# charlie-foxtrot/RTLSDR-Airband

Measured on AMD Instinct MI355X. Metric: IQ Msamples/sec channelized+demodulated per node; % HBM roofline, higher is better.
Workload: dtype i8x3->i32->f32 (stage 1), f32 (stage 2)

## Files before the change

### rtlsdr-airband_amd/_build.py

```python
from __future__ import annotations

import os
import subprocess
import sys

import hashlib

HERE = os.path.dirname(os.path.abspath(__file__))
CSRC = os.path.join(HERE, "csrc")
ARCH = "gfx950"
EXTRA = os.environ.get("AIRBAND_EXTRA_DEFINES", "").split()
TAG = os.environ.get("AIRBAND_BUILD_TAG") or (hashlib.sha1(" ".join(EXTRA).encode()).hexdigest()[:8] if EXTRA else "")
OBJ = os.path.join(HERE, "build" + ("_exp_" + TAG if EXTRA else ""))
LIB = os.path.join(HERE, "libairband_hip" + ("_exp_" + TAG if EXTRA else "") + ".so")

DEVICE_FLAGS = ["-Xclang", "-target-feature", "-Xclang", "-packed-fp32-ops"]

HIP_SOURCES = {
    "channelizer_fft.hip": ["-O3"],
    "channelizer_dft.hip": ["-O3"],
    "channelizer_dft_wide.hip": ["-O3"],
    "channelizer_f32.hip": ["-O3"],
    "misc_kernels.hip": ["-O3", "-ffp-contract=off"],
    "demod.hip": ["-O3", "-ffp-contract=off", "-fhip-fp32-correctly-rounded-divide-sqrt"],
    "gate.hip": ["-O3"],
    "airband_hip.cpp": ["-O2", "-x", "hip"],
}
HOST_SOURCES = {"params.cpp": ["-O2", "-ffp-contract=off", "-fno-fast-math"]}


def _newer(src: str, dst: str) -> bool:
    if not os.path.exists(dst):
        return True
    t = os.path.getmtime(dst)
    deps = [src, os.path.abspath(__file__)] + [os.path.join(CSRC, f) for f in os.listdir(CSRC) if f.endswith(".h")] + [os.path.join(HERE, "..", "include", "airband_hip.h")]
    return any(os.path.getmtime(d) > t for d in deps)


def _run(cmd):
    r = subprocess.run(cmd, stdout=subprocess.PIPE, stderr=subprocess.STDOUT, text=True)
    if r.returncode != 0:
        sys.stderr.write(" ".join(cmd) + "\n" + r.stdout)
        raise RuntimeError("build failed: " + " ".join(cmd[:3]))
    return r.stdout


LLVM_BIN = "/opt/rocm/lib/llvm/bin"
FORBIDDEN = r"^\s+v_pk_(mul|fma|add)_f32"


def device_disassembly(lib: str):
    import re
    import shutil
    import tempfile

    def tool(name):
        t = os.path.join(LLVM_BIN, name)
        t = t if os.path.exists(t) else shutil.which(name)
        if not t:
            raise RuntimeError("the packed-f32 guard needs " + name + " (ROCm's llvm/bin)")
        return t

    units = []
    with tempfile.TemporaryDirectory(prefix="airband_fatbin_") as d:
        fat = os.path.join(d, "fat.bin")
        _run([tool("llvm-objcopy"), "--dump-section", ".hip_fatbin=" + fat, lib, os.devnull])
        blob = open(fat, "rb").read()
        magic = b"__CLANG_OFFLOAD_BUNDLE__"
        starts = [m.start() for m in re.finditer(re.escape(magic), blob)]
        if not starts:
            raise RuntimeError("no offload bundle in .hip_fatbin of " + lib)
        for n, (a, b) in enumerate(zip(starts, starts[1:] + [len(blob)])):
            piece, co = os.path.join(d, "bundle%d.bin" % n), os.path.join(d, "unit%d.co" % n)
            open(piece, "wb").write(blob[a:b])
            _run([tool("clang-offload-bundler"), "--unbundle", "--type=o", "--targets=hipv4-amdgcn-amd-amdhsa--" + ARCH, "--input=" + piece, "--output=" + co])
            text = _run([tool("llvm-objdump"), "-d", co])
            units.append((re.findall(r"^[0-9a-f]+ <(\w+)>:", text, re.M), text))
    return units


def check_no_packed_f32(lib: str) -> int:
    import re

    n = 0
    for kernels, text in device_disassembly(lib):
        for line in text.split("\n"):
            if re.match(r"^\s+[sv]_\w+|^\s+(ds|global|buffer|flat|scratch)_\w+", line):
                n += 1
                if re.match(FORBIDDEN, line):
                    raise RuntimeError("packed-f32 instruction in the device code of %s (kernels of the unit: %s ...): %s" % (lib, ", ".join(kernels[:3]), line.strip()))
    if n < 100000 and not EXTRA:
        raise RuntimeError("packed-f32 guard: only %d device instructions found in %s" % (n, lib))
    return n


def build(force: bool = False, verbose: bool = False) -> str:
    sources = [os.path.join(CSRC, name) for name in list(HIP_SOURCES) + list(HOST_SOURCES)]
    if not force and all(os.path.exists(s) for s in sources) and not any(_newer(s, LIB) for s in sources):
        return LIB
    os.makedirs(OBJ, exist_ok=True)
    hipcc = os.environ.get("HIPCC", "/opt/rocm/bin/hipcc")
    objs = []
    changed = False
    for name, flags in HIP_SOURCES.items():
        src = os.path.join(CSRC, name)
        if not os.path.exists(src):
            continue
        obj = os.path.join(OBJ, name + ".o")
        objs.append(obj)
        if force or _newer(src, obj):
            info = ["-DAB_BUILD_DEFINES=\"%s\"" % " ".join(EXTRA)] if name == "airband_hip.cpp" else []
            cmd = [hipcc, "--offload-arch=" + ARCH, "-std=c++17", "-fPIC", "-Wall", "-Wno-unused-function"] + flags + DEVICE_FLAGS + EXTRA + info + ["-c", src, "-o", obj]
            if verbose:
                print(" ".join(cmd))
            _run(cmd)
            changed = True
    for name, flags in HOST_SOURCES.items():
        src = os.path.join(CSRC, name)
        obj = os.path.join(OBJ, name + ".o")
        objs.append(obj)
        if force or _newer(src, obj):
            cmd = ["g++", "-std=c++17", "-fPIC", "-Wall"] + flags + ["-c", src, "-o", obj]
            if verbose:
                print(" ".join(cmd))
            _run(cmd)
            changed = True
    if changed or not os.path.exists(LIB):
        cmd = [hipcc, "--offload-arch=" + ARCH, "-shared", "-fPIC", "-o", LIB] + objs + ["-Wl,--no-undefined"]
        if verbose:
            print(" ".join(cmd))
        tmp = LIB + ".unchecked"
        cmd[cmd.index("-o") + 1] = tmp
        _run(cmd)
        if not any("+packed-fp32-ops" in e for e in EXTRA):
            try:
                check_no_packed_f32(tmp)
            except Exception:
                os.unlink(tmp)
                raise
        os.replace(tmp, LIB)
    return LIB


if __name__ == "__main__":
    print(build(force="--force" in sys.argv, verbose=True))
```

### rtlsdr-airband_amd/csrc/demod.hip

```cpp
#include <hip/hip_runtime.h>

#include <cstdlib>
#include <type_traits>

#include "common.h"
#include "kernels.h"
#include "squelch_fsm.h"
#include "exact_math.h"

namespace airband {

namespace {

#if !defined(AB_NEEDED_NOW)
#if defined(__HIPCC__)
#define AB_NEEDED_NOW(...) asm volatile("" ::__VA_ARGS__)
#define AB_V(x) "v"(x)
#else
#define AB_NEEDED_NOW(...) ((void)0)
#define AB_V(x) 0
#endif
#endif
#if !defined(AB_SCHED_FENCE)
#if defined(__has_builtin) && __has_builtin(__builtin_amdgcn_sched_barrier)
// ... 57 lines not shown
    int stride;
    int j0;
    const float* stage_base;
    const int* ext_of;
    float* out_wave;
    int wave_stride;
    bool coop;
    int* skip_of;
};

struct RowZero {
    int held;
    bool run_open;
    bool batch_open;
};
__device__ __forceinline__ bool row_skip_run(const RowZero& z) { return (z.held & 2) && !z.run_open; }
__device__ __forceinline__ void row_run_done(RowZero& z) {
    z.batch_open = z.batch_open || z.run_open;
    z.run_open = false;
}

__device__ __forceinline__ void wave_tail_copy(float* row, int B) {
    typedef float v4f __attribute__((ext_vector_type(4)));
    const v4f* src = reinterpret_cast<const v4f*>(row + B);
    v4f* dst = reinterpret_cast<v4f*>(row);
    static_assert((AB_AGC_EXTRA / 4) % 5 == 0, "whole rounds");
#pragma unroll 1
    for (int c = 0; c < AB_AGC_EXTRA / 4; c += 5) {
        const v4f t0 = src[c], t1 = src[c + 1], t2 = src[c + 2], t3 = src[c + 3], t4 = src[c + 4];
        dst[c] = t0; dst[c + 1] = t1; dst[c + 2] = t2; dst[c + 3] = t3; dst[c + 4] = t4;
    }
}

__device__ __forceinline__ void row_tail_copy(RowZero& z, float* row, int B) {
    if ((z.held & 3) != 3) wave_tail_copy(row, B);
    z.held = (z.held & 2) ? 3 : 0;
}

__device__ __forceinline__ void wave_flush(const WaveRow& w, RowZero& z, int n = RUN) {
    const bool skip = row_skip_run(z);
    row_run_done(z);
    if (w.coop) {
        const int lane = threadIdx.x & 63, q = lane & 7;
        AB_LOCKSTEP();
        w.skip_of[lane] = skip ? 1 : 0;
        AB_LOCKSTEP();
        if (4 * q < n) {
#pragma unroll
            for (int i = 0; i < 8; i++) {
                const int c = i * 8 + (lane >> 3);
                if (w.skip_of[c]) continue;
                const float* src = w.stage_base + (4 * q) * OSTRIDE + c;
                float4* dst = reinterpret_cast<float4*>(w.out_wave + (long)w.ext_of[c] * w.wave_stride + AB_OUT_PAD + AB_AGC_EXTRA + w.j0 + 4 * q);
                *dst = make_float4(src[0], src[OSTRIDE], src[2 * OSTRIDE], src[3 * OSTRIDE]);
            }
        }
        AB_LOCKSTEP();
        return;
    }
    if (skip) return;
    float4* dst = reinterpret_cast<float4*>(w.row + AB_AGC_EXTRA + w.j0);
#pragma unroll
    for (int q = 0; q < RUN / 4; q++)
        if (4 * q < n)
        dst[q] = make_float4(w.staged[(4 * q) * w.stride], w.staged[(4 * q + 1) * w.stride], w.staged[(4 * q + 2) * w.stride], w.staged[(4 * q + 3) * w.stride]);
}

__device__ __forceinline__ void emit_sample(const DemodArgs& a, const ChanConst& cc, OutRegs& o, const WaveRow& w, RowZero& z, float2* iqout, uint8_t* trace, int j, bool audio, bool fade,
                                            bool tone, int state, float out, float re, float im, bool write_iq_always) {
    constexpr long S = AB_SLOT_BLOCK;
    if (AB_UNLIKELY(fade)) {
        z.run_open = true;
        float prev = w.row[j];
#pragma nounroll
        for (int k = j + 1; k < j + AB_AGC_EXTRA; k++) {
            prev = prev * 0.94f;
            const int i = k - AB_AGC_EXTRA - w.j0;
            if (i >= 0)
                w.staged[i * w.stride] = prev;
            else
                w.row[k] = prev;
        }
    }
    const bool open = audio && tone;
    if (open) {
        if (cc.flags & AB_F_NOTCH) {
            o.nx0 = o.nx1; o.nx1 = o.nx2; o.nx2 = out;
            o.ny0 = o.ny1; o.ny1 = o.ny2;
            o.ny2 = cc.notch_d0 * o.nx2 - cc.notch_d1 * o.nx1 + cc.notch_d0 * o.nx0 + cc.notch_d1 * o.ny1 - cc.notch_d2 * o.ny0;
            out = o.ny2;
        }
        out *= cc.ampfactor;
        out = (out != out) ? 0.0f : __builtin_amdgcn_fmed3f(out, -1.0f, 1.0f);
        o.axc = '*';
        z.run_open = true;
    } else {
        out = 0.0f;
    }
    w.staged[(j - w.j0) * w.stride] = out;
    if (cc.flags & AB_F_IQ_OUT) {
        if (open) {
            if (write_iq_always) iqout[(long)j * S] = make_float2(re, im);
        } else {
            iqout[(long)j * S] = make_float2(0.0f, 0.0f);
        }
    }
    if (trace) trace[(long)j * S] = (uint8_t)((state & 7) | (open ? 8 : 0) | (audio ? 16 : 0) | (((cc.flags & AB_F_CTCSS) && tone) ? 32 : 0));
}

constexpr unsigned KIND_MASK = AB_F_NFM | AB_F_RAW_IQ | AB_F_LOWPASS | AB_F_CTCSS | AB_F_IQ_OUT;
template <int KIND>
struct KindBits {
    static constexpr unsigned value = KIND == AB_KIND_NFM           ? (AB_F_NFM | AB_F_RAW_IQ)
                                      : KIND == AB_KIND_NFM_LOWPASS ? (AB_F_NFM | AB_F_RAW_IQ | AB_F_LOWPASS)
                                      : KIND == AB_KIND_NFM_CTCSS   ? (AB_F_NFM | AB_F_RAW_IQ | AB_F_CTCSS)
                                                                    : 0u;
};

template <int KIND, bool WAVE_HAS_CTCSS, int W>
__device__ __forceinline__ void demod_wave(const DemodArgs& a, ChanConst cc, ChanState* sp, int slot, const float2* lut, float* ostage, const int* ext_of, int* skip_of, const int* slot_of,
                                           bool full_block) {
    const int lane = threadIdx.x & 63;
    constexpr long S = AB_SLOT_BLOCK;
    const int R = a.ring_rows, B = a.wave_batch;
    const bool valid = (cc.flags & AB_F_VALID) != 0;
    if (KIND != AB_KIND_GENERIC) cc.flags = (cc.flags & ~KIND_MASK) | KindBits<KIND>::value;

    if (!valid) return;

    const bool nfm = cc.flags & AB_F_NFM, raw_iq = cc.flags & AB_F_RAW_IQ, lowpass = cc.flags & AB_F_LOWPASS;
    const lmask m_am = ab_ballot(!nfm), m_raw_iq = ab_ballot(raw_iq);

    Lane L;
    L.m_lowpass = ab_ballot(lowpass);
    L.m_manual = ab_ballot((cc.flags & AB_F_MANUAL) != 0);
    L.manual_level = cc.sq_manual_level;
    L.normal_ratio = cc.sq_normal_ratio;
    L.flappy_ratio = cc.sq_flappy_ratio;
    L.m_flappy_lower = ab_ballot(cc.sq_flappy_ratio < cc.sq_normal_ratio);
    L.sqbuf = a.sqbuf + ab_ring_base(slot, AB_SQ_BUF);
    L.S = S;
    L.prefetched_delay = (KIND == AB_KIND_NFM_LOWPASS);
    L.track_delay_line = (KIND == AB_KIND_NFM_LOWPASS || KIND == AB_KIND_GENERIC);
    L.may_post_filter = (KIND == AB_KIND_NFM_LOWPASS || KIND == AB_KIND_GENERIC);
    L.all_lowpass = (KIND == AB_KIND_NFM_LOWPASS);
    L.shadow_delay = (KIND == AB_KIND_NFM_LOWPASS);

    SqRegs s;
    sq_load(s, L, sp, true);
    const bool aligned4 = ((s.sample_count + 1u) & 3u) == 0u;
    SqShadow sh = {sp->sh_nf, sp->sh_cap, sp->sh_capped};
    const bool first_batch = a.tail_copy == 0;
    s.dly = KIND == AB_KIND_NFM_LOWPASS ? sp->sh_dly : 0.0f;
    float agc = sp->agcavgfast, pr = sp->pr, pj = sp->pj, prev_out = sp->prev_waveout;
    unsigned dm_phi = sp->dm_phi;
    OutRegs o;
    o.nx0 = sp->nx[0]; o.nx1 = sp->nx[1]; o.nx2 = sp->nx[2]; o.ny0 = sp->ny[0]; o.ny1 = sp->ny[1]; o.ny2 = sp->ny[2];
    o.axc = ' ';
    float lxr1 = sp->lxr[1], lxr2 = sp->lxr[2], lxi1 = sp->lxi[1], lxi2 = sp->lxi[2];
    float lyr1 = sp->lyr[1], lyr2 = sp->lyr[2], lyi1 = sp->lyi[1], lyi2 = sp->lyi[2];

    const float one_minus_alpha = 1.0f - cc.alpha;
    const float div_lo = cc.lp_rgain != 0.0f ? AB_DIV_CONST_LO : __builtin_inff();

    float* mag = a.mag + ab_tile_base(slot, R / AB_TILE_ROWS);
    const float2* iqin = a.iq + ab_tile_base(slot, R / AB_TILE_ROWS);
    const int ext = a.slot_to_ext[slot];
    WaveRow wrow;
    wrow.row = a.out_wave + (long)ext * a.wave_stride + AB_OUT_PAD;
    wrow.stride = OSTRIDE;
    wrow.j0 = 0;
    wrow.stage_base = ostage;
    wrow.ext_of = ext_of;
    wrow.out_wave = a.out_wave;
    wrow.wave_stride = a.wave_stride;
    wrow.coop = full_block;
    wrow.skip_of = skip_of;
    lmask audio_seen = 0;
    RowZero rz = {sp->row_zero, false, false};
    float2* iqout = a.iq_out + ab_ring_base(slot, B);
    uint8_t* trace = a.trace ? a.trace + ab_ring_base(slot, B) : nullptr;
    wrow.staged = ostage + lane;
    if (!WAVE_HAS_CTCSS && a.tail_copy) row_tail_copy(rz, wrow.row, B);
    constexpr bool PACKED = WAVE_HAS_CTCSS && KIND == AB_KIND_NFM_CTCSS;
    float2* ct_af = (WAVE_HAS_CTCSS && !PACKED) ? a.ct_af + (long)(slot - a.ct_gen_first_block * 64) * B : nullptr;
    unsigned* ct_ap = PACKED ? a.ct_ap + (long)(slot - a.ct_pk_first_block * 64) * a.ct_pk_pitch : nullptr;
    constexpr int HAND_RUN = PACKED ? RUN : 16;
    float2* hand_base = reinterpret_cast<float2*>(ostage);
    float2* hand = hand_base + lane;
    unsigned* handw_base = reinterpret_cast<unsigned*>(ostage);
    unsigned* handw = handw_base + lane;
    auto ct_row = [&](int c) { return a.ct_af + (long)(slot_of[c] - a.ct_gen_first_block * 64) * B; };
    auto ct_roww = [&](int c) { return a.ct_ap + (long)(slot_of[c] - a.ct_pk_first_block * 64) * a.ct_pk_pitch; };
    auto hand_flush = [&](int n, int jstart) {
        if (PACKED) {
            if (full_block) {
                const int q = lane & 7;
                AB_LOCKSTEP();
                if (4 * q < n) {
#pragma unroll
                    for (int i0 = 0; i0 < 8; i0++) {
#if defined(AB_FLUSH_REVERSED)
                        const int i = 7 - i0;
#else
                        const int i = i0;
#endif
                        const int c = i * 8 + (lane >> 3);
                        const unsigned* src = handw_base + (4 * q) * OSTRIDE + c;
                        *reinterpret_cast<uint4*>(ct_roww(c) + jstart + 4 * q) = make_uint4(src[0], src[OSTRIDE], src[2 * OSTRIDE], src[3 * OSTRIDE]);
                    }
                }
                AB_LOCKSTEP();
            } else {
                for (int i = 0; i < n; i += 4)
                    *reinterpret_cast<uint4*>(ct_ap + jstart + i) = make_uint4(handw[i * OSTRIDE], handw[(i + 1) * OSTRIDE], handw[(i + 2) * OSTRIDE], handw[(i + 3) * OSTRIDE]);
            }
            return;
        }
        if (full_block) {
            const int q = lane & 7;
            AB_LOCKSTEP();
            if (2 * q < n) {
#pragma unroll
                for (int i = 0; i < 8; i++) {
                    const int c = i * 8 + (lane >> 3);
                    const float2 p0 = hand_base[(2 * q) * OSTRIDE + c], p1 = hand_base[(2 * q + 1) * OSTRIDE + c];
                    *reinterpret_cast<float4*>(ct_row(c) + jstart + 2 * q) = make_float4(p0.x, p0.y, p1.x, p1.y);
                }
            }
            AB_LOCKSTEP();
        } else {
            for (int i = 0; i < n; i += 2) {
                const float2 p0 = hand[i * OSTRIDE], p1 = hand[(i + 1) * OSTRIDE];
                *reinterpret_cast<float4*>(ct_af + jstart + i) = make_float4(p0.x, p0.y, p1.x, p1.y);
            }
        }
    };

    constexpr int GS = 4;
    constexpr int GQ = GS / 4;
#if defined(AB_MASKED_DELAY)
    constexpr bool MASKD = KIND == AB_KIND_AM || KIND == AB_KIND_NFM || KIND == AB_KIND_NFM_CTCSS;
#define AB_MD_PARAM , const int r
#define AB_MD_ARG(r) , r
#else
#define AB_MD_PARAM
#define AB_MD_ARG(r)
#endif
    struct Group {
        float4 mc[GQ], md[GQ], c01[GQ], c23[GQ], q01[GQ], q23[GQ];
#if defined(AB_MASKED_DELAY)
        lmask real;
#endif
    };
    auto fetch = [&](Group& q, int j0, int tail0) {
#if defined(AB_MASKED_DELAY)
        const lmask need = MASKD ? (~s.cC & s.active) : ~(lmask)0;
        const bool real_lane = !MASKD || ab_lane(need);
        q.real = need;
#endif
#pragma unroll
        for (int g = 0; g < GQ; g++) {
            const int rc = ring_row(a.row0 + AB_AGC_EXTRA + j0 + 4 * g, R);
#if defined(AB_MASKED_DELAY)
            const int rd = real_lane ? ring_row(a.row0 + j0 + 4 * g, R) : rc;
#else
            const int rd = ring_row(a.row0 + j0 + 4 * g, R);
#endif
            if (!nfm) {
                q.mc[g] = *reinterpret_cast<const float4*>(mag + ab_tile_off(rc));
                q.md[g] = *reinterpret_cast<const float4*>(mag + ab_tile_off(rd));
            } else {
                const float4* cp = reinterpret_cast<const float4*>(iqin + ab_tile_off(rc));
                q.c01[g] = cp[0];
                q.c23[g] = cp[1];
            }
            if (raw_iq) {
                const float4* qp = reinterpret_cast<const float4*>(iqin + ab_tile_off(rd));
                q.q01[g] = qp[0];
                q.q23[g] = qp[1];
            }
        }
        (void)tail0;
    };
#if defined(AB_MASKED_DELAY)
    float g_md[4] = {0.0f, 0.0f, 0.0f, 0.0f}, g_qr[4] = {0.0f, 0.0f, 0.0f, 0.0f}, g_qi[4] = {0.0f, 0.0f, 0.0f, 0.0f};
    lmask g_real = 0;
    int g_jq = 0;
    auto refetch = [&](const lmask miss) {
        if (ab_lane(miss)) {
            const int rd = ring_row(a.row0 + g_jq, R);
            if (!nfm) {
                const float4 v = *reinterpret_cast<const float4*>(mag + ab_tile_off(rd));
                g_md[0] = v.x; g_md[1] = v.y; g_md[2] = v.z; g_md[3] = v.w;
            } else {
                const float4* qp = reinterpret_cast<const float4*>(iqin + ab_tile_off(rd));
                const float4 u = qp[0], v = qp[1];
                g_qr[0] = u.x; g_qi[0] = u.y; g_qr[1] = u.z; g_qi[1] = u.w;
                g_qr[2] = v.x; g_qi[2] = v.y; g_qr[3] = v.z; g_qi[3] = v.w;
            }
        }
        g_real |= miss;
    };
#endif
    auto touch = [&](const Group& q) {
#pragma unroll
        for (int g = 0; g < GQ; g++) {
            if (!nfm) AB_NEEDED_NOW(AB_V(q.mc[g].x), AB_V(q.mc[g].y), AB_V(q.mc[g].z), AB_V(q.mc[g].w), AB_V(q.md[g].x), AB_V(q.md[g].y), AB_V(q.md[g].z), AB_V(q.md[g].w));
            else AB_NEEDED_NOW(AB_V(q.c01[g].x), AB_V(q.c01[g].y), AB_V(q.c01[g].z), AB_V(q.c01[g].w), AB_V(q.c23[g].x), AB_V(q.c23[g].y), AB_V(q.c23[g].z), AB_V(q.c23[g].w));
            if (raw_iq) AB_NEEDED_NOW(AB_V(q.q01[g].x), AB_V(q.q01[g].y), AB_V(q.q01[g].z), AB_V(q.q01[g].w), AB_V(q.q23[g].x), AB_V(q.q23[g].y), AB_V(q.q23[g].z), AB_V(q.q23[g].w));
        }
    };
    auto tail_in = [&](int n) {
// ... 263 lines not shown
                const float xr0 = xr1, xi0 = xi1;
                xr1 = xr2; xi1 = xi2;
                ab_div_const2(tr, ti, cc.lp_gain, cc.lp_rgain, div_lo, xr2, xi2);
                const float yr0 = yr1, yi0 = yi1;
                yr1 = yr2; yi1 = yi2;
                yr2 = (xr0 + xr2) + (2.0f * xr1) + (cc.lp_yc0 * yr0) + (cc.lp_yc1 * yr1);
                yi2 = (xi0 + xi2) + (2.0f * xi1) + (cc.lp_yc0 * yi0) + (cc.lp_yc1 * yi1);
                re = yr2;
                im = yi2;
                fmag = ab_sqrt_rn(re * re + im * im);
            }
            fre[r] = re;
            fim[r] = im;
            if (ab_any(filt)) {
                const float delayed = t.dly;
                const lmask run = filt & ~(t.cOg & ab_ballot(t.delay < AB_SQ_BUF));
                const lmask seed = run & t.cOg & ab_ballot(t.delay == AB_SQ_BUF);
                float full = ab_lane(seed) ? delayed : t.post_full, capped = ab_lane(seed) ? delayed : t.post_capped;
                t.using_post |= run;
                sq_avg(t.cap, full, capped, fmag);
                t.post_full = ab_lane(run) ? full : t.post_full;
                t.post_capped = ab_lane(run) ? capped : t.post_capped;
                bad |= run & ab_ballot(capped < delayed);
            }
            AB_SCHED_FENCE();
        }
        bad |= t.cC & ~ab_ballot(t.closed_count < 1000u) & t.recent_nz;
        if (AB_UNLIKELY(ab_any(bad & t.active))) return false;
        s = t;
        dm_phi = phi;
        lxr1 = xr1; lxr2 = xr2; lxi1 = xi1; lxi2 = xi2; lyr1 = yr1; lyr2 = yr2; lyi1 = yi1; lyi2 = yi2;
        const bool audio = ab_lane(sq_should_audio(s));
        const int state = !a.trace ? 0 : sq_cur(s);
#pragma unroll
        for (int r = 0; r < 4; r++) {
            float out = 0.0f;
            const float re = fre[r], im = fim[r];
            if (audio) {
                if (!(cc.flags & AB_F_QUADRI)) {
                    const float nbj = -pj;
                    const float cr = re * pr - im * nbj;
                    const float cj = im * pr + re * nbj;
                    out = (float)((double)fast_atan2_dev(cj, cr) * 0.31830988618379067154);
                } else {
                    out = (float)((double)((pr * im - re * pj) / (re * re + im * im + 1.0f)) * 0.31830988618379067154);
                }
                pr = re;
                pj = im;
                agc = agc * 0.995f + out * 0.005f;
                out -= agc;
                out = out * one_minus_alpha + prev_out * cc.alpha;
                prev_out = out;
            }
            emit_sample(a, cc, o, wrow, rz, iqout, trace, jq + r, audio, false, true, state, out, re, im, true);
            AB_SCHED_FENCE();
        }
        return true;
    };
    auto group = [&](const Group& q, int j0) {
#pragma unroll
        for (int g = 0; g < GQ; g++) {
            float mcs[4], mds[4] = {0.0f, 0.0f, 0.0f, 0.0f}, qr[4] = {0.0f, 0.0f, 0.0f, 0.0f}, qi[4] = {0.0f, 0.0f, 0.0f, 0.0f};
            if (!nfm) {
                mcs[0] = q.mc[g].x; mcs[1] = q.mc[g].y; mcs[2] = q.mc[g].z; mcs[3] = q.mc[g].w;
                mds[0] = q.md[g].x; mds[1] = q.md[g].y; mds[2] = q.md[g].z; mds[3] = q.md[g].w;
            } else {
                const float pw[4] = {q.c01[g].x * q.c01[g].x + q.c01[g].y * q.c01[g].y, q.c01[g].z * q.c01[g].z + q.c01[g].w * q.c01[g].w,
                                     q.c23[g].x * q.c23[g].x + q.c23[g].y * q.c23[g].y, q.c23[g].z * q.c23[g].z + q.c23[g].w * q.c23[g].w};
                ab_sqrt_rn4(pw, mcs);
            }
            if (raw_iq) {
                qr[0] = q.q01[g].x; qi[0] = q.q01[g].y; qr[1] = q.q01[g].z; qi[1] = q.q01[g].w;
                qr[2] = q.q23[g].x; qi[2] = q.q23[g].y; qr[3] = q.q23[g].z; qi[3] = q.q23[g].w;
            }
            const int jq = j0 + 4 * g;
            if (KIND == AB_KIND_NFM_LOWPASS) {
                const unsigned c0 = s.sample_count;
                const float dpw[4] = {qr[0] * qr[0] + qi[0] * qi[0], qr[1] * qr[1] + qi[1] * qi[1], qr[2] * qr[2] + qi[2] * qi[2], qr[3] * qr[3] + qi[3] * qi[3]};
                float dmag[4];
                ab_sqrt_rn4(dpw, dmag);
#pragma unroll
                for (int r = 0; r < 4; r++) {
                    const int j = jq + r;
                    mds[r] = (first_batch && j < 101) ? 0.0f : sq_shadow_value(sh);
                    if (!(first_batch && j < AB_AGC_EXTRA)) sq_shadow_step(sh, L, dmag[r], c0 + (unsigned)r + 2u);
                }
            }
            if ((jq % RUN) == 0) wrow.j0 = jq;
#if defined(AB_MASKED_DELAY)
            if (MASKD) {
#pragma unroll
                for (int r = 0; r < 4; r++) { g_md[r] = mds[r]; g_qr[r] = qr[r]; g_qi[r] = qi[r]; }
                g_real = q.real;
                g_jq = jq;
                const lmask want0 = nfm ? ((~s.cC | ~s.nC) & ~s.cA & s.active) : (s.cO | s.cCg | s.nO | s.nCg);
                const lmask miss0 = want0 & ~g_real;
                if (AB_UNLIKELY(ab_any(miss0))) refetch(miss0);
                if (SPEC4 && AB_LIKELY(aligned4 && sq_stable4(s))) {
                    if (AB_LIKELY(sq_raw_stable4(s, L, mcs))) {
                        stable_tail4(jq, mcs, g_md, g_qr, g_qi);
                        continue;
                    }
                }
#pragma unroll
                for (int r = 0; r < 4; r++) sample(jq + r, mcs[r], g_md[r], g_qr[r], g_qi[r], r == 0, r);
                continue;
            }
#endif
            if (SPEC4 && AB_LIKELY(aligned4 && sq_stable4(s))) {
                if (AB_LIKELY(sq_raw_stable4(s, L, mcs))) {
                    stable_tail4(jq, mcs, mds, qr, qi);
                    continue;
                }
            }
            if (SPEC4_LP && AB_LIKELY(aligned4 && sq_stable4(s))) {
                if (AB_LIKELY(lp_stable4(jq, mcs, mds, qr, qi))) continue;
            }
#pragma unroll
            for (int r = 0; r < 4; r++) sample(jq + r, mcs[r], mds[r], qr[r], qi[r], r == 0 AB_MD_ARG(r));
        }
    };
    auto flush = [&](int j0) {
        if (!WAVE_HAS_CTCSS && ((j0 + GS) % RUN) == 0) wave_flush(wrow, rz);
        if (WAVE_HAS_CTCSS && ((j0 + GS) % HAND_RUN) == 0) hand_flush(HAND_RUN, j0 + GS - HAND_RUN);
    };

    Group qa, qb;
    fetch(qa, 0, s.tail);
    touch(qa);
    for (int j0 = 0; j0 < B; j0 += 2 * GS) {
#if !defined(AB_REGROUP_FREE)
        if (W > 1 && a.regroup != 2) __syncthreads();
#endif
        fetch(qb, j0 + GS, tail_in(GS));
        group(qa, j0);
        touch(qb);
        flush(j0);
        fetch(qa, j0 + 2 * GS < B ? j0 + 2 * GS : B - GS, tail_in(GS));
        group(qb, j0 + GS);
        touch(qa);
        flush(j0 + GS);
    }

    if (!WAVE_HAS_CTCSS && (B % RUN) != 0) wave_flush(wrow, rz, B % RUN);
    if (WAVE_HAS_CTCSS && (B % HAND_RUN) != 0) hand_flush(B % HAND_RUN, B - B % HAND_RUN);
    if (!WAVE_HAS_CTCSS) {
        if (o.axc != ' ') sp->active_counter++;
        sp->axc_prev = sp->axc;
        sp->axc = o.axc;
        a.out_axc[ext] = (uint8_t)o.axc;
        sp->nx[0] = o.nx0; sp->nx[1] = o.nx1; sp->nx[2] = o.nx2; sp->ny[0] = o.ny0; sp->ny[1] = o.ny1; sp->ny[2] = o.ny2;
        sp->row_zero = rz.batch_open ? 0 : ((rz.held & 1) | 2);
    }
    sp->agcavgfast = agc; sp->pr = pr; sp->pj = pj; sp->prev_waveout = prev_out; sp->dm_phi = dm_phi;
    if (KIND == AB_KIND_NFM_LOWPASS) { sp->sh_nf = sh.nf; sp->sh_cap = sh.cap; sp->sh_capped = sh.capped; sp->sh_dly = s.dly; }
    if (KIND == AB_KIND_GENERIC) sp->sh_dly = sq_delayed(s, L);
    sq_store(s, L, sp, B);
    if (WAVE_HAS_CTCSS) a.sq_key[slot] = ab_lane(audio_seen) ? 1 : 0;
    sp->lxr[1] = lxr1; sp->lxr[2] = lxr2; sp->lxi[1] = lxi1; sp->lxi[2] = lxi2;
    sp->lyr[1] = lyr1; sp->lyr[2] = lyr2; sp->lyi[1] = lyi1; sp->lyi[2] = lyi2;
}

constexpr int TONE_GROUP = 50;

}

#ifndef AB_AM_WAVES_N
#define AB_AM_WAVES_N 4
#endif
constexpr int AB_DEMOD_WAVES = 3, AB_AM_WAVES = AB_AM_WAVES_N, AB_FRONT_WAVES = 3;

constexpr int AB_REGROUP_WAVES = 4;
constexpr int WAVE_LDS_FLOATS = RUN * OSTRIDE + 3 * 64;

template <int W>
__device__ __forceinline__ int wg_regroup(int key, int wave, int lane, int home, int nb, int* slot_at, int* wcnt) {
    const lmask m0 = __ballot(key == 0), m1 = __ballot(key == 1), m2 = __ballot(key == 2);
    if (lane == 0) {
        wcnt[2 * wave] = __builtin_popcountll(m0);
        wcnt[2 * wave + 1] = __builtin_popcountll(m1);
    }
    __syncthreads();
    int tot0 = 0, tot1 = 0, off0 = 0, off1 = 0;
#pragma unroll
    for (int w = 0; w < W; w++) {
        const int c0 = wcnt[2 * w], c1 = wcnt[2 * w + 1];
        tot0 += c0;
        tot1 += c1;
        off0 += w < wave ? c0 : 0;
        off1 += w < wave ? c1 : 0;
    }
    const lmask below = lane == 0 ? 0ull : (~0ull >> (64 - lane));
    const int at = key == 0   ? off0 + __builtin_popcountll(m0 & below)
                   : key == 1 ? tot0 + off1 + __builtin_popcountll(m1 & below)
                   : key == 2 ? tot0 + tot1 + (wave * 64 - off0 - off1) + __builtin_popcountll(m2 & below)
                              : -1;
    if (at >= 0) slot_at[at] = home;
    __syncthreads();
    const int p = wave * 64 + lane;
    return p < nb * 64 ? slot_at[p] : -1;
}

template <int KIND, bool WAVE_HAS_CTCSS, int W>
__device__ __forceinline__ void demod_block(const DemodArgs& a, int first_block, int n_blocks, float* lds_demod) {
    const int lane = threadIdx.x & 63;
    const int wave = W > 1 ? __builtin_amdgcn_readfirstlane((int)(threadIdx.x >> 6)) : 0;
    float2* lut = reinterpret_cast<float2*>(lds_demod);
    if (KIND != AB_KIND_AM) {
        for (int i = threadIdx.x; i < 257; i += 64 * W) lut[i] = make_float2(a.sin_lut[i], a.cos_lut[i]);
        if (W == 1) __syncthreads();
    }
    float* areas = reinterpret_cast<float*>(lut + (KIND == AB_KIND_AM ? 0 : 258));
    float* ostage = areas + wave * WAVE_LDS_FLOATS;
    int* ext_of = reinterpret_cast<int*>(ostage + RUN * OSTRIDE);
    int* skip_of = ext_of + 64;
    int* slot_of = skip_of + 64;
    int slot;
    if (W == 1) {
        slot = (first_block + blockIdx.x) * 64 + lane;
        if (a.perm) slot = a.perm[slot];
    } else {
        int* slot_at = reinterpret_cast<int*>(areas + W * WAVE_LDS_FLOATS);
        int* wcnt = slot_at + W * 64;
        const int block0 = first_block + blockIdx.x * W;
        const int left = first_block + n_blocks - block0, nb = left < W ? left : W;
        const int home = (block0 + wave) * 64 + lane;
        int key = 3;
        if (wave < nb) {
            const ChanState* hp = a.cs + home;
            const bool valid = (a.cc[home].flags & AB_F_VALID) != 0;
            bool busy = valid && (hp->cur != AB_ST_CLOSED || hp->next != AB_ST_CLOSED);
            if (a.regroup == 2) {
                constexpr int G = (KIND == AB_KIND_AM || KIND == AB_KIND_GENERIC) ? 4 : 2;
                const lmask any_busy = __ballot(busy);
                const lmask gmask = ((1ull << G) - 1ull) << (lane & ~(G - 1));
                busy = (any_busy & gmask) != 0ull;
            }
            key = !valid ? 2 : busy ? 0 : 1;
        }
        slot = wg_regroup<W>(key, wave, lane, home, nb, slot_at, wcnt);
        if (slot < 0) return;
    }
    const ChanConst cc = a.cc[slot];
    ext_of[lane] = a.slot_to_ext[slot];
    slot_of[lane] = slot;
    const bool full_block = __ballot((cc.flags & AB_F_VALID) != 0) == ~0ull;
    if (W == 1) __syncthreads();
    else AB_LOCKSTEP_FENCED();
    demod_wave<KIND, WAVE_HAS_CTCSS, W>(a, cc, a.cs + slot, slot, lut, ostage, ext_of, skip_of, slot_of, full_block);
}

template <int KIND, bool WAVE_HAS_CTCSS, int W>
__global__ __launch_bounds__(64 * W, KIND == AB_KIND_AM ? AB_AM_WAVES : KIND == AB_KIND_NFM_CTCSS ? AB_FRONT_WAVES : AB_DEMOD_WAVES) void demod_kernel(DemodArgs a, int first_block, int n_blocks) {
    AB_DYNAMIC_LDS(float, lds_demod);
    demod_block<KIND, WAVE_HAS_CTCSS, W>(a, first_block, n_blocks, lds_demod);
}

constexpr int AB_PERM_WAVES = 16;
template <int G>
__global__ __launch_bounds__(64 * AB_PERM_WAVES) void regroup_perm_kernel(DemodArgs a, int first_block, int n_blocks) {
    __shared__ int slot_at[AB_PERM_WAVES * 64];
    __shared__ int wcnt[AB_PERM_WAVES * 2];
    const int lane = threadIdx.x & 63;
    const int wave = __builtin_amdgcn_readfirstlane((int)(threadIdx.x >> 6));
    const int block0 = first_block + blockIdx.x * AB_PERM_WAVES;
    const int left = first_block + n_blocks - block0, nb = left < AB_PERM_WAVES ? left : AB_PERM_WAVES;
    const int home = (block0 + wave) * 64 + lane;
    int key = 3;
    if (wave < nb) {
        const ChanState* hp = a.cs + home;
        const bool valid = (a.cc[home].flags & AB_F_VALID) != 0;
        const bool busy1 = valid && (hp->cur != AB_ST_CLOSED || hp->next != AB_ST_CLOSED);
        const lmask any_busy = __ballot(busy1);
        const lmask gmask = ((1ull << G) - 1ull) << (lane & ~(G - 1));
        key = !valid ? 2 : (any_busy & gmask) != 0ull ? 0 : 1;
    }
    const int slot = wg_regroup<AB_PERM_WAVES>(key, wave, lane, home, nb, slot_at, wcnt);
    if (slot >= 0) a.perm[home] = slot;
}

#if defined(AB_TONE_WAVES8)
#define AB_TONE_RESIDENCY __attribute__((amdgpu_waves_per_eu(8, 8)))
#else
#define AB_TONE_RESIDENCY
#endif
template <bool PACKED>
__global__ __launch_bounds__(256) AB_TONE_RESIDENCY void tone_kernel(DemodArgs a, int first_block, int n_blocks) {
    __shared__ float power[4][64];
    __shared__ __attribute__((aligned(16))) float xs_all[4][64];
    const int wave = __builtin_amdgcn_readfirstlane((int)((blockIdx.x * blockDim.x + threadIdx.x) >> 6));
    const int lane = threadIdx.x & 63;
    if (wave >= n_blocks * 64) return;
    const int slot = first_block * 64 + wave;
    const unsigned flags = a.cc[slot].flags;
    if (!(flags & AB_F_VALID) || !(flags & AB_F_CTCSS)) return;
    const ChanConst cc = a.cc[slot];
    ChanState* sp = a.cs + slot;
    float* scratch = power[threadIdx.x >> 6];
    float* xs = xs_all[threadIdx.x >> 6];
    const int B = a.wave_batch, NG = B / TONE_GROUP;
    int enough0 = sp->ct_enough[0], enough1 = sp->ct_enough[1], count0 = sp->ct_count[0], count1 = sp->ct_count[1];
    int has0 = sp->ct_has_tone[0], has1 = sp->ct_has_tone[1];
    unsigned found0 = sp->ct_found[0], found1 = sp->ct_found[1], nf0 = sp->ct_not_found[0], nf1 = sp->ct_not_found[1];
    const int n0 = cc.ct_ntones[0], n1 = cc.ct_ntones[1], win0 = cc.ct_window[0], win1 = cc.ct_window[1];
    const float* ctab = a.ct_coeff + (long)cc.ct_slot * 2 * AB_MAX_TONES;
    float* qtab = a.ct_q + (long)cc.ct_slot * 4 * AB_MAX_TONES;
    const bool merged = n0 + n1 <= 64;
    const int fi = merged ? lane - n1 : lane;
    const bool t0 = fi >= 0 && fi < n0, t1 = lane < n1;
    const int fbase = merged ? n1 : 0;
    const float c0 = t0 ? ctab[fi] : 0.0f, c1 = t1 ? ctab[AB_MAX_TONES + lane] : 0.0f;
    float q1f = t0 ? qtab[fi] : 0.0f, q2f = t0 ? qtab[AB_MAX_TONES + fi] : 0.0f;
    float q1s = t1 ? qtab[2 * AB_MAX_TONES + lane] : 0.0f, q2s = t1 ? qtab[3 * AB_MAX_TONES + lane] : 0.0f;

    const long blk = (wave >> 6) + (first_block - a.ct_first_block);
    if (!a.sq_key[slot]) {
        const unsigned long long standing = ((sp->ct_enough[1] ? sp->ct_has_tone[1] : sp->ct_has_tone[0]) != 0) ? ~0ull : 0ull;
        unsigned long long* mp = a.ct_mask + (blk * (a.wave_batch / TONE_GROUP)) * AB_SLOT_BLOCK + (wave & 63);
        if (lane < a.wave_batch / TONE_GROUP) mp[(long)lane * AB_SLOT_BLOCK] = standing;
        return;
    }
    const long hrow = wave + (long)(first_block - (PACKED ? a.ct_pk_first_block : a.ct_gen_first_block)) * 64;
    const float2* af = PACKED ? nullptr : a.ct_af + hrow * B;
    const unsigned* ap = PACKED ? a.ct_ap + hrow * a.ct_pk_pitch : nullptr;
    unsigned long long* maskp = a.ct_mask + (blk * NG) * AB_SLOT_BLOCK + (wave & 63);
    constexpr int DEPTH = 10;
    const int ldlane = lane < TONE_GROUP ? lane : TONE_GROUP - 1;
    auto fetch = [&](int g) {
        const int i = (g < NG ? g : NG - 1) * TONE_GROUP + ldlane;
        if (PACKED) return make_float2(__uint_as_float(ap[i]), 0.0f);
        return af[i];
    };
    float2 ahead[DEPTH];
#pragma unroll
    for (int k = 0; k < DEPTH; k++) ahead[k] = fetch(k);
    unsigned long long verdict[DEPTH];
    auto step = [&](const int g, const float2 got, unsigned long long& mask_out) {
        float2 cur = lane < TONE_GROUP ? got : make_float2(0.0f, 0.0f);
        if (PACKED) {
            const unsigned w = lane < TONE_GROUP ? __float_as_uint(got.x) : HAND_IDLE;
            const bool au = hand_is_audio(w);
            cur = make_float2(au ? __uint_as_float(w) : 0.0f, __uint_as_float(au ? FL_AUDIO : ((w & 1u) ? FL_RESET : 0u)));
        }
        const float ax = cur.x;
        const unsigned fl = __float_as_uint(cur.y);
        unsigned long long mask = 0;
        const bool idle = __ballot((fl & (FL_AUDIO | FL_RESET)) != 0) == 0ull;
        const bool all_audio = __ballot(lane < TONE_GROUP && (fl & (FL_AUDIO | FL_RESET)) != FL_AUDIO) == 0ull;
        if (idle) {
            mask = (enough1 ? has1 : has0) ? ~0ull : 0ull;
        } else if (all_audio && count1 + TONE_GROUP < win1 && (enough1 || count0 + TONE_GROUP < win0)) {
#if defined(AB_TONE_READLANE)
            if (enough1) {
                for (int u = 0; u < TONE_GROUP; u++) {
                    const float x = __uint_as_float(__builtin_amdgcn_readlane(__float_as_uint(ax), u));
                    const float q0 = c1 * q1s - q2s + x;
                    q2s = q1s;
                    q1s = q0;
                }
            } else {
                for (int u = 0; u < TONE_GROUP; u++) {
                    const float x = __uint_as_float(__builtin_amdgcn_readlane(__float_as_uint(ax), u));
                    const float q0 = c1 * q1s - q2s + x;
                    q2s = q1s;
                    q1s = q0;
                    const float p0 = c0 * q1f - q2f + x;
                    q2f = q1f;
                    q1f = p0;
                }
                count0 += TONE_GROUP;
            }
#else
            AB_LOCKSTEP_FENCED();
            xs[lane] = ax;
            AB_LOCKSTEP_FENCED();
            static_assert(TONE_GROUP % 4 == 2 && TONE_GROUP + 2 <= 64, "twelve quads and one pair; the last quad read covers two parked zeros");
            const float4* xs4 = reinterpret_cast<const float4*>(xs);
            float4 v = xs4[0];
            if (enough1) {
#pragma unroll 2
                for (int u4 = 0; u4 < TONE_GROUP / 4; u4++) {
                    const float4 nxt = xs4[u4 + 1];
                    const float x4[4] = {v.x, v.y, v.z, v.w};
#pragma unroll
                    for (int r = 0; r < 4; r++) {
                        const float q0 = c1 * q1s - q2s + x4[r];
                        q2s = q1s;
                        q1s = q0;
                    }
                    v = nxt;
                }
                const float x2[2] = {v.x, v.y};
#pragma unroll
                for (int r = 0; r < 2; r++) {
                    const float q0 = c1 * q1s - q2s + x2[r];
                    q2s = q1s;
                    q1s = q0;
                }
// ... 403 lines not shown
```

### rtlsdr-airband_amd/csrc/squelch_fsm.h

```cpp
#ifndef AIRBAND_CSRC_SQUELCH_FSM_H
#define AIRBAND_CSRC_SQUELCH_FSM_H

#include "common.h"

namespace airband {

typedef unsigned long long lmask;

#if defined(__HIPCC__)
#define AB_FSM_FN __device__ __forceinline__
AB_FSM_FN lmask ab_ballot(bool b) { return __ballot(b); }
AB_FSM_FN bool ab_lane(lmask m) { return __builtin_amdgcn_inverse_ballot_w64(m); }
AB_FSM_FN bool ab_any(lmask m) { return m != 0ull; }
AB_FSM_FN unsigned ab_uniform(unsigned v) { return (unsigned)__builtin_amdgcn_readfirstlane((int)v); }
#define AB_LIKELY(x) __builtin_expect(!!(x), 1)
#define AB_UNLIKELY(x) __builtin_expect(!!(x), 0)
AB_FSM_FN bool ab_rare(lmask m) { return AB_UNLIKELY(m != 0ull); }
#else
#define AB_FSM_FN static inline
AB_FSM_FN lmask ab_ballot(bool b) { return b ? 1ull : 0ull; }
AB_FSM_FN bool ab_lane(lmask m) { return (m & 1ull) != 0ull; }
AB_FSM_FN bool ab_any(lmask m) { return (m & 1ull) != 0ull; }
AB_FSM_FN unsigned ab_uniform(unsigned v) { return v; }
#define AB_LIKELY(x) (x)
// ... 143 lines not shown
    const float lo = s.noise_floor < s.pre_capped ? s.noise_floor : s.pre_capped;
    s.noise_floor = s.noise_floor * decay + lo * fresh + 1e-6f;
    s.cap = ab_lane(L.m_manual) ? 1.5f * L.manual_level : 1.5f * L.normal_ratio * s.noise_floor;
    s.lvl = sq_level_compute(s, L);
}

struct SqShadow {
    float nf, cap, capped;
};
AB_FSM_FN float sq_shadow_value(const SqShadow& h) { return h.capped * 0.9f; }
AB_FSM_FN void sq_shadow_step(SqShadow& h, const Lane& L, float x, unsigned phase) {
    if (((phase - 101u) & 15u) == 0u) {
        const float decay = 0.97f;
        const float fresh = (float)(1.0 - (double)0.97f);
        const float lo = h.nf < h.capped ? h.nf : h.capped;
        h.nf = h.nf * decay + lo * fresh + 1e-6f;
        h.cap = ab_lane(L.m_manual) ? 1.5f * L.manual_level : 1.5f * L.normal_ratio * h.nf;
    }
    const float decay = 0.99f;
    const float fresh = (float)(1.0 - (double)0.99f);
    const float xf = x * fresh;
    const float v = h.capped * decay + xf;
    const float vm = v < h.cap ? v : h.cap;
    h.capped = (h.capped >= h.cap && x >= h.cap) ? h.cap : vm;
}

AB_FSM_FN void sq_raw_quiet(SqRegs& s, const Lane& L, float x, float dly_new, bool may_sweep = true) {
    const lmask below = ab_ballot(s.closed_count < 1000u);
    s.closed_count += ab_lane(s.cC & below) ? 1u : 0u;
    if (L.track_delay_line) {
        s.tail = s.tail + 1 == AB_SQ_BUF ? 0 : s.tail + 1;
        s.head = s.head + 1 == AB_SQ_BUF ? 0 : s.head + 1;
    }
    s.dly = dly_new;
    s.sample_count++;
    if (may_sweep && AB_UNLIKELY((s.sample_count & 15u) == 0u)) sq_noise_floor(s, L);
    sq_avg(s.cap, s.pre_full, s.pre_capped, x);
    sq_delay_line_push(s, L);
    const lmask sig = sq_has_signal(s, L);
    const lmask low = s.cO & ab_ballot(!(x >= s.lvl));
    const int run = s.low_count + 1;
    const int idle = ab_lane(s.cO) ? 0 : s.low_count;
    s.low_count = ab_lane(low) ? run : idle;
    const lmask abort_now = low & ab_ballot(s.low_count >= 88);
    const lmask to_closing = s.cO & ~sig, to_opening = s.cC & sig;
    const lmask any_req = to_closing | to_opening | abort_now;
    s.nA = abort_now;
    s.nCg = to_closing & ~abort_now;
    s.nOg = to_opening;
    s.nO &= ~any_req;
    s.nC &= ~any_req;
    s.quiet = !ab_any((any_req | sq_saturated(s)) & s.active);
}

AB_FSM_FN bool sq_stable4(const SqRegs& s) {
    const lmask moving = (s.nC ^ s.cC) | (s.nOg ^ s.cOg) | (s.nCg ^ s.cCg) | (s.nA ^ s.cA) | (s.nO ^ s.cO);
    const lmask timed = s.cOg | s.cCg | s.cA;
    const lmask expiring = timed & ab_ballot(s.delay > 197 - 1 - 4);
    return !ab_any((moving | expiring | sq_saturated(s)) & s.active);
}
AB_FSM_FN bool sq_raw_stable4(SqRegs& s, const Lane& L, const float* x) {
    SqRegs t = s;
    const unsigned cc4 = t.closed_count + (ab_lane(t.cC) ? 4u : 0u);
    t.closed_count = cc4 < 1000u ? cc4 : 1000u;
    t.delay += ab_lane(t.cOg | t.cCg | t.cA) ? 4 : 0;
    t.sample_count += 1u;
    if (AB_UNLIKELY((t.sample_count & 15u) == 0u)) sq_noise_floor(t, L);
    t.sample_count += 3u;
    const lmask counting = t.cOg | t.cCg | t.cO;
    const lmask want = t.cO;
    const lmask care = t.cO | t.cC;
    lmask bad = 0;
    for (int r = 0; r < 4; r++) {
        sq_avg(t.cap, t.pre_full, t.pre_capped, x[r]);
        const lmask sig = ab_ballot(t.pre_capped >= t.lvl);
        const lmask low = counting & ab_ballot(!(x[r] >= t.lvl));
        const int run = t.low_count + 1;
        const int idle = ab_lane(counting) ? 0 : t.low_count;
        t.low_count = ab_lane(low) ? run : idle;
        bad |= ((sig ^ want) & care) | (low & ab_ballot(t.low_count >= 88));
    }
    bad |= t.cC & ~ab_ballot(t.closed_count < 1000u) & t.recent_nz;
    if (AB_UNLIKELY(ab_any(bad & t.active))) return false;
    s = t;
    return true;
}

AB_FSM_FN lmask sq_raw_full(SqRegs& s, const Lane& L, float x, float dly_new) {
    const lmask went_closed = sq_advance(s, L);
    s.dly = dly_new;
    s.sample_count++;
    if ((s.sample_count & 15u) == 0u) sq_noise_floor(s, L);
    sq_avg(s.cap, s.pre_full, s.pre_capped, x);
    sq_delay_line_push(s, L);
    const lmask sig = sq_has_signal(s, L);
    const lmask to_closing = s.cO & ~sig;
    const lmask to_opening = s.cC & sig;
    const lmask counting = s.cOg | s.cCg | s.cO;
    const lmask low = counting & ab_ballot(!(x >= s.lvl));
    const int run = s.low_count + 1;
    const int idle = ab_lane(counting) ? 0 : s.low_count;
    s.low_count = ab_lane(low) ? run : idle;
    const lmask abort_now = low & ab_ballot(s.low_count >= 88);
    const lmask any_req = to_closing | to_opening | abort_now;
    if (ab_any(any_req)) {
        s.nC = (s.nC & ~any_req) | (abort_now & s.cOg);
        s.nA = (s.nA & ~any_req) | (abort_now & ~s.cOg);
        s.nCg = (s.nCg & ~any_req) | (to_closing & ~abort_now);
        s.nOg = (s.nOg & ~any_req) | (to_opening & ~abort_now);
        s.nO &= ~any_req;
    }
    s.quiet = sq_is_quiet(s);
    return went_closed;
}

AB_FSM_FN lmask sq_raw(SqRegs& s, const Lane& L, float x, float dly_new) {
    if (AB_LIKELY(s.quiet)) {
        sq_raw_quiet(s, L, x, dly_new);
        return 0;
    }
    return sq_raw_full(s, L, x, dly_new);
}

AB_FSM_FN lmask sq_should_filter(const SqRegs& s) { return (sq_has_pre(s) | ~s.cC) & ~s.cA & s.active; }
AB_FSM_FN lmask sq_should_audio(const SqRegs& s) { return s.cO | s.cCg; }
AB_FSM_FN lmask sq_first_open(const SqRegs& s) { return ~s.cO & s.nO; }
AB_FSM_FN lmask sq_last_open(const SqRegs& s) { return (s.cCg & s.nC) | (~s.cA & s.nA); }

AB_FSM_FN void sq_filtered(SqRegs& s, const Lane& L, lmask filt, float x) {
    filt &= L.m_lowpass;
    if (!ab_any(filt)) return;
    const float delayed = sq_delayed(s, L);
    const lmask run = filt & ~(s.cOg & ab_ballot(s.delay < AB_SQ_BUF));
    const lmask seed = run & s.cOg & ab_ballot(s.delay == AB_SQ_BUF);
    float full = ab_lane(seed) ? delayed : s.post_full, capped = ab_lane(seed) ? delayed : s.post_capped;
    s.using_post |= run;
    sq_avg(s.cap, full, capped, x);
    s.post_full = ab_lane(run) ? full : s.post_full;
    s.post_capped = ab_lane(run) ? capped : s.post_capped;
    const lmask close = run & ab_ballot(capped < delayed);
    if (ab_rare(close)) {
        s.nC = (s.nC & ~close) | (close & ~s.cO);
        s.nCg = (s.nCg & ~close) | (close & s.cO);
        s.nOg &= ~close;
        s.nA &= ~close;
        s.nO &= ~close;
        s.quiet = false;
    }
}

AB_FSM_FN void sq_load(SqRegs& s, const Lane& L, const ChanState* sp, bool valid) {
    s.active = ab_ballot(valid);
    s.noise_floor = sp->noise_floor; s.cap = sp->cap; s.pre_full = sp->pre_full; s.pre_capped = sp->pre_capped;
    s.post_full = sp->post_full; s.post_capped = sp->post_capped;
    s.using_post = ab_ballot(valid && sp->using_post != 0);
    sq_set_next(s, valid ? sp->next : -1);
    sq_set_cur(s, valid ? sp->cur : -1);
    s.delay = sp->delay; s.low_count = sp->low_count;
    s.head = (int)ab_uniform((unsigned)sp->head); s.tail = (int)ab_uniform((unsigned)sp->tail);
    s.sample_count = ab_uniform(sp->sample_count); s.open_count = sp->open_count;
    s.flappy_count = sp->flappy_count; s.recent_open = sp->recent_open; s.closed_count = sp->closed_count;
    s.recent_nz = ab_ballot(valid && sp->recent_open != 0u);
    s.lvl = sq_level_compute(s, L);
    s.dly = 0.0f;
    s.quiet = sq_is_quiet(s);
}

AB_FSM_FN void sq_store(const SqRegs& s, const Lane& L, ChanState* sp, int samples) {
    sp->noise_floor = s.noise_floor; sp->cap = s.cap; sp->pre_full = s.pre_full; sp->pre_capped = s.pre_capped;
    sp->post_full = s.post_full; sp->post_capped = s.post_capped;
    sp->using_post = ab_lane(s.using_post) ? 1 : 0; sp->next = sq_next(s); sp->cur = sq_cur(s); sp->delay = s.delay; sp->low_count = s.low_count;
    int head = s.head, tail = s.tail;
    if (!L.track_delay_line) {
        head = (head + samples) % AB_SQ_BUF;
        tail = (tail + samples) % AB_SQ_BUF;
    }
    sp->head = head; sp->tail = tail; sp->sample_count = s.sample_count; sp->open_count = s.open_count;
    sp->flappy_count = s.flappy_count; sp->recent_open = s.recent_open; sp->closed_count = s.closed_count;
}

}

#endif
```

Baseline: 1.570 million.

## Trim AM demod kernel state and LDS to fit more waves per block

For the AM kernel, per-channel state that only FM or lowpass paths use (raw-IQ phase, lowpass delay lines, post-filter squelch levels) is no longer loaded or stored, and the slot index shares LDS with the skip array unless CTCSS is active. This shrinks per-wave LDS and register pressure, which lets the AM wave count per block go from 4 to 5. A build-time guard now enforces a VGPR cap and zero scratch on the AM kernel. The risk is that aliasing skip_of and slot_of is only correct if the skip data is dead whenever CTCSS uses the slots.

Result: no change. 1.569 million (-0.1%).

```diff
diff --git a/rtlsdr-airband_amd/_build.py b/rtlsdr-airband_amd/_build.py
--- a/rtlsdr-airband_amd/_build.py
+++ b/rtlsdr-airband_amd/_build.py
@@ -49,7 +49,7 @@
 FORBIDDEN = r"^\s+v_pk_(mul|fma|add)_f32"
 
 
-def device_disassembly(lib: str):
+def device_disassembly(lib: str, listing=("llvm-objdump", "-d")):
     import re
     import shutil
     import tempfile
@@ -74,7 +74,7 @@
             piece, co = os.path.join(d, "bundle%d.bin" % n), os.path.join(d, "unit%d.co" % n)
             open(piece, "wb").write(blob[a:b])
             _run([tool("clang-offload-bundler"), "--unbundle", "--type=o", "--targets=hipv4-amdgcn-amd-amdhsa--" + ARCH, "--input=" + piece, "--output=" + co])
-            text = _run([tool("llvm-objdump"), "-d", co])
+            text = _run([tool(listing[0])] + list(listing[1:]) + [co])
             units.append((re.findall(r"^[0-9a-f]+ <(\w+)>:", text, re.M), text))
     return units
 
@@ -92,6 +92,34 @@
     if n < 100000 and not EXTRA:
         raise RuntimeError("packed-f32 guard: only %d device instructions found in %s" % (n, lib))
     return n
+
+
+AM_KERNEL = "demod_kernelILi0E"
+AM_MAX_VGPRS = 96
+
+
+def kernel_resources(lib: str):
+    import re
+
+    out = {}
+    for _, text in device_disassembly(lib, listing=("llvm-readobj", "--notes")):
+        for entry in re.split(r"^\s+- \.agpr_count:", text, flags=re.M)[1:]:
+            sym = re.search(r"^\s+\.symbol:\s+'?([\w.$]+?)\.kd'?\s*$", entry, re.M)
+            if not sym:
+                continue
+            field = lambda name: int(re.search(r"^\s+\." + name + r":\s+(\d+)", entry, re.M).group(1))
+            out[sym.group(1)] = dict(vgpr=field("vgpr_count"), scratch=field("private_segment_fixed_size"), lds=field("group_segment_fixed_size"))
+    return out
+
+
+def check_am_kernel_lean(lib: str):
+    res = {k: v for k, v in kernel_resources(lib).items() if AM_KERNEL in k}
+    if not res:
+        raise RuntimeError("AM-kernel guard: no %s* kernel found in %s" % (AM_KERNEL, lib))
+    for k, v in res.items():
+        if v["scratch"] != 0 or v["vgpr"] > AM_MAX_VGPRS:
+            raise RuntimeError("AM-kernel guard: %s uses %d VGPRs and %d bytes of scratch per lane (at most %d and 0)" % (k, v["vgpr"], v["scratch"], AM_MAX_VGPRS))
+    return res
 
 
 def build(force: bool = False, verbose: bool = False) -> str:
@@ -138,6 +166,12 @@
             except Exception:
                 os.unlink(tmp)
                 raise
+        if not EXTRA:
+            try:
+                check_am_kernel_lean(tmp)
+            except Exception:
+                os.unlink(tmp)
+                raise
         os.replace(tmp, LIB)
     return LIB
 
diff --git a/rtlsdr-airband_amd/csrc/demod.hip b/rtlsdr-airband_amd/csrc/demod.hip
--- a/rtlsdr-airband_amd/csrc/demod.hip
+++ b/rtlsdr-airband_amd/csrc/demod.hip
@@ -233,13 +233,19 @@
     SqShadow sh = {sp->sh_nf, sp->sh_cap, sp->sh_capped};
     const bool first_batch = a.tail_copy == 0;
     s.dly = KIND == AB_KIND_NFM_LOWPASS ? sp->sh_dly : 0.0f;
-    float agc = sp->agcavgfast, pr = sp->pr, pj = sp->pj, prev_out = sp->prev_waveout;
-    unsigned dm_phi = sp->dm_phi;
+    constexpr bool HAS_RAW_IQ = KIND != AB_KIND_AM;
+    constexpr bool HAS_LOWPASS = KIND == AB_KIND_NFM_LOWPASS || KIND == AB_KIND_GENERIC;
+    float agc = sp->agcavgfast, pr = 0.0f, pj = 0.0f, prev_out = 0.0f;
+    unsigned dm_phi = 0u;
+    if (HAS_RAW_IQ) { pr = sp->pr; pj = sp->pj; prev_out = sp->prev_waveout; dm_phi = sp->dm_phi; }
     OutRegs o;
     o.nx0 = sp->nx[0]; o.nx1 = sp->nx[1]; o.nx2 = sp->nx[2]; o.ny0 = sp->ny[0]; o.ny1 = sp->ny[1]; o.ny2 = sp->ny[2];
     o.axc = ' ';
-    float lxr1 = sp->lxr[1], lxr2 = sp->lxr[2], lxi1 = sp->lxi[1], lxi2 = sp->lxi[2];
-    float lyr1 = sp->lyr[1], lyr2 = sp->lyr[2], lyi1 = sp->lyi[1], lyi2 = sp->lyi[2];
+    float lxr1 = 0.0f, lxr2 = 0.0f, lxi1 = 0.0f, lxi2 = 0.0f, lyr1 = 0.0f, lyr2 = 0.0f, lyi1 = 0.0f, lyi2 = 0.0f;
+    if (HAS_LOWPASS) {
+        lxr1 = sp->lxr[1]; lxr2 = sp->lxr[2]; lxi1 = sp->lxi[1]; lxi2 = sp->lxi[2];
+        lyr1 = sp->lyr[1]; lyr2 = sp->lyr[2]; lyi1 = sp->lyi[1]; lyi2 = sp->lyi[2];
+    }
 
     const float one_minus_alpha = 1.0f - cc.alpha;
     const float div_lo = cc.lp_rgain != 0.0f ? AB_DIV_CONST_LO : __builtin_inff();
@@ -809,13 +815,16 @@
         sp->nx[0] = o.nx0; sp->nx[1] = o.nx1; sp->nx[2] = o.nx2; sp->ny[0] = o.ny0; sp->ny[1] = o.ny1; sp->ny[2] = o.ny2;
         sp->row_zero = rz.batch_open ? 0 : ((rz.held & 1) | 2);
     }
-    sp->agcavgfast = agc; sp->pr = pr; sp->pj = pj; sp->prev_waveout = prev_out; sp->dm_phi = dm_phi;
+    sp->agcavgfast = agc;
+    if (HAS_RAW_IQ) { sp->pr = pr; sp->pj = pj; sp->prev_waveout = prev_out; sp->dm_phi = dm_phi; }
     if (KIND == AB_KIND_NFM_LOWPASS) { sp->sh_nf = sh.nf; sp->sh_cap = sh.cap; sp->sh_capped = sh.capped; sp->sh_dly = s.dly; }
     if (KIND == AB_KIND_GENERIC) sp->sh_dly = sq_delayed(s, L);
     sq_store(s, L, sp, B);
     if (WAVE_HAS_CTCSS) a.sq_key[slot] = ab_lane(audio_seen) ? 1 : 0;
-    sp->lxr[1] = lxr1; sp->lxr[2] = lxr2; sp->lxi[1] = lxi1; sp->lxi[2] = lxi2;
-    sp->lyr[1] = lyr1; sp->lyr[2] = lyr2; sp->lyi[1] = lyi1; sp->lyi[2] = lyi2;
+    if (HAS_LOWPASS) {
+        sp->lxr[1] = lxr1; sp->lxr[2] = lxr2; sp->lxi[1] = lxi1; sp->lxi[2] = lxi2;
+        sp->lyr[1] = lyr1; sp->lyr[2] = lyr2; sp->lyi[1] = lyi1; sp->lyi[2] = lyi2;
+    }
 }
 
 constexpr int TONE_GROUP = 50;
@@ -823,12 +832,12 @@
 }
 
 #ifndef AB_AM_WAVES_N
-#define AB_AM_WAVES_N 4
+#define AB_AM_WAVES_N 5
 #endif
 constexpr int AB_DEMOD_WAVES = 3, AB_AM_WAVES = AB_AM_WAVES_N, AB_FRONT_WAVES = 3;
 
 constexpr int AB_REGROUP_WAVES = 4;
-constexpr int WAVE_LDS_FLOATS = RUN * OSTRIDE + 3 * 64;
+constexpr int WAVE_LDS_FLOATS = RUN * OSTRIDE + 2 * 64;
 
 template <int W>
 __device__ __forceinline__ int wg_regroup(int key, int wave, int lane, int home, int nb, int* slot_at, int* wcnt) {
@@ -871,7 +880,7 @@
     float* ostage = areas + wave * WAVE_LDS_FLOATS;
     int* ext_of = reinterpret_cast<int*>(ostage + RUN * OSTRIDE);
     int* skip_of = ext_of + 64;
-    int* slot_of = skip_of + 64;
+    int* slot_of = skip_of;
     int slot;
     if (W == 1) {
         slot = (first_block + blockIdx.x) * 64 + lane;
@@ -900,7 +909,7 @@
     }
     const ChanConst cc = a.cc[slot];
     ext_of[lane] = a.slot_to_ext[slot];
-    slot_of[lane] = slot;
+    if (WAVE_HAS_CTCSS) slot_of[lane] = slot;
     const bool full_block = __ballot((cc.flags & AB_F_VALID) != 0) == ~0ull;
     if (W == 1) __syncthreads();
     else AB_LOCKSTEP_FENCED();
diff --git a/rtlsdr-airband_amd/csrc/squelch_fsm.h b/rtlsdr-airband_amd/csrc/squelch_fsm.h
--- a/rtlsdr-airband_amd/csrc/squelch_fsm.h
+++ b/rtlsdr-airband_amd/csrc/squelch_fsm.h
@@ -319,7 +319,7 @@
 AB_FSM_FN void sq_load(SqRegs& s, const Lane& L, const ChanState* sp, bool valid) {
     s.active = ab_ballot(valid);
     s.noise_floor = sp->noise_floor; s.cap = sp->cap; s.pre_full = sp->pre_full; s.pre_capped = sp->pre_capped;
-    s.post_full = sp->post_full; s.post_capped = sp->post_capped;
+    s.post_full = L.may_post_filter ? sp->post_full : 0.0f; s.post_capped = L.may_post_filter ? sp->post_capped : 0.0f;
     s.using_post = ab_ballot(valid && sp->using_post != 0);
     sq_set_next(s, valid ? sp->next : -1);
     sq_set_cur(s, valid ? sp->cur : -1);
@@ -335,7 +335,7 @@
 
 AB_FSM_FN void sq_store(const SqRegs& s, const Lane& L, ChanState* sp, int samples) {
     sp->noise_floor = s.noise_floor; sp->cap = s.cap; sp->pre_full = s.pre_full; sp->pre_capped = s.pre_capped;
-    sp->post_full = s.post_full; sp->post_capped = s.post_capped;
+    if (L.may_post_filter) { sp->post_full = s.post_full; sp->post_capped = s.post_capped; }
     sp->using_post = ab_lane(s.using_post) ? 1 : 0; sp->next = sq_next(s); sp->cur = sq_cur(s); sp->delay = s.delay; sp->low_count = s.low_count;
     int head = s.head, tail = s.tail;
     if (!L.track_delay_line) {
```
